# Sreyan88/audio-ssl

Measured on AMD Instinct MI355X. Metric: upstream clips/sec (1s@16kHz, 64-mel), higher is better.
Workload: dtype bf16; 1 GPU; delores-m upstream step (log-mel + 2 views + q/k conv encoders + MoCo + 3 Barlow heads + bwd + SGD), 1 s @ 16 kHz, 64 mel, batch 512/GPU, queue 65536; global_batch=512, parallelism=dp1

## Files before the change

### audio-ssl_amd/csrc/augment.hip

```cpp
#include "common.h"

namespace {

constexpr float F32_EPS = 1.1920928955078125e-07f;
constexpr float F32_MAX = 3.4028234663852886e+38f;

__global__ __launch_bounds__(256) void clip_moments_kernel(const float* __restrict__ x, double* __restrict__ mom, int n) {
    __shared__ double sh[16];
    const float* p = x + (long)blockIdx.x * n;
    double s = 0.0, q = 0.0;
    for (int i = threadIdx.x; i < n; i += 256) { const double v = p[i]; s += v; q += v * v; }
    s = block_sum(s, sh);
    q = block_sum(q, sh);
    if (threadIdx.x == 0) { mom[2 * blockIdx.x] = s; mom[2 * blockIdx.x + 1] = q; }
}

__device__ __forceinline__ float chain64(float v, float x_mine, double r_mine, float& keep) {
    const int rlo = __double2loint(r_mine), rhi = __double2hiint(r_mine);
#pragma unroll
    for (int c = 0; c < 64; ++c) {
        const float x = __int_as_float(__builtin_amdgcn_readlane(__float_as_int(x_mine), c));
        const double r = __hiloint2double(__builtin_amdgcn_readlane(rhi, c), __builtin_amdgcn_readlane(rlo, c));
        v = v + (float)((double)(x - v) * r);
        keep = ((int)(threadIdx.x & 63) == c) ? v : keep;
    }
    return v;
}

__global__ __launch_bounds__(128) void runnorm_scan_kernel(const double* __restrict__ mom, int B, int n_elem, long long* state_i,
                                                           float* state_f, float* __restrict__ mu_out, float* __restrict__ sd_out) {
    extern __shared__ __attribute__((aligned(16))) double sm[];
    double* rn = sm;
    float* m_s = reinterpret_cast<float*>(rn + B);
    float* mu_s = m_s + B;
    float* v_s = mu_s + B;
    float* s2_s = v_s + B;
    const long long n0 = state_i[0], max_update = state_i[1];
    const double inv = 1.0 / (double)n_elem;
    const int tid = threadIdx.x, wave = tid >> 6, lane = tid & 63;
    const bool big = n0 + B > (1 << 24);
    for (int c = tid; c < B; c += 128) {
        m_s[c] = (float)(mom[2 * c] * inv);
        const long long n = n0 + c;
        rn[c] = (n > 0 && n < max_update) ? (big ? (double)(float)n : 1.0 / (double)(float)n) : 0.0;
    }
    float mu = state_f[0], s2 = state_f[1];
    const bool first = n0 == 0 && max_update > 0;
    __syncthreads();
    const int nblk = (B + 63) / 64;
    for (int k = 0; k <= nblk; ++k) {
        if (wave == 0 && k < nblk) {
            const int c0 = 64 * k, c = c0 + lane;
            if (!big) {
                if (k == 0 && first) mu = m_s[0];
                float keep = 0.f;
                mu = chain64(mu, c < B ? m_s[c] : 0.f, c < B ? rn[c] : 0.0, keep);
                if (c < B) mu_s[c] = keep;
            } else if (lane == 0) {
                int i = c0;
                const int c1 = min(c0 + 64, B);
                if (i == 0 && first) { mu = m_s[0]; mu_s[0] = mu; i = 1; }
                for (; i < c1; ++i) { if (rn[i] != 0.0) mu = mu + (m_s[i] - mu) / (float)rn[i]; mu_s[i] = mu; }
            }
        }
        if (wave == 1 && k >= 1) {
            const int c0 = 64 * (k - 1), c1 = min(c0 + 64, B), c = c0 + lane;
            float v = 0.f;
            if (c < c1) {
                const double ex = mom[2 * c] * inv, ex2 = mom[2 * c + 1] * inv, mud = (double)mu_s[c];
                v = (float)(ex2 - 2.0 * mud * ex + mud * mud);
            }
            if (!big) {
                if (k == 1 && first) s2 = __int_as_float(__builtin_amdgcn_readlane(__float_as_int(v), 0));
                float keep = 0.f;
                s2 = chain64(s2, v, c < c1 ? rn[c] : 0.0, keep);
                if (c < c1) s2_s[c] = keep;
            } else {
                if (c < c1) v_s[c] = v;
                __threadfence_block();
                if (lane == 0) {
                    int i = c0;
                    if (i == 0 && first) { s2 = v_s[0]; s2_s[0] = s2; i = 1; }
                    for (; i < c1; ++i) { if (rn[i] != 0.0) s2 = s2 + (v_s[i] - s2) / (float)rn[i]; s2_s[i] = s2; }
                }
            }
        }
        __syncthreads();
    }
    for (int c = tid; c < B; c += 128) {
        mu_out[c] = mu_s[c];
        sd_out[c] = fminf(fmaxf(sqrtf(s2_s[c]), F32_EPS), F32_MAX);
    }
    if (tid == 0) {
        long long upd = max_update - n0;
        upd = upd < 0 ? 0 : (upd > B ? B : upd);
        state_i[0] = n0 + upd;
        state_f[0] = mu_s[B - 1];
        state_f[1] = s2_s[B - 1];
    }
}

__global__ __launch_bounds__(256) void aug_normalize_kernel(const float* __restrict__ x, const float* __restrict__ mu,
                                                            const float* __restrict__ sd, float* __restrict__ bank,
                                                            long slot0, int R, int n) {
    const int c = blockIdx.y;
    const float m = mu[c], s = sd[c];
    const float* src = x + (long)c * n;
    float* dst = bank + ((slot0 + c) % R) * (long)n;
    for (int i = blockIdx.x * 256 + threadIdx.x; i < n; i += gridDim.x * 256) dst[i] = (src[i] - m) / s;
}

__device__ __forceinline__ void cubic_coeffs(float t, float* c) {
    const float A = -0.75f;
    float x = t + 1.f;
    c[0] = ((A * x - 5.f * A) * x + 8.f * A) * x - 4.f * A;
    x = t;
    c[1] = ((A + 2.f) * x - (A + 3.f)) * x * x + 1.f;
    x = 1.f - t;
    c[2] = ((A + 2.f) * x - (A + 3.f)) * x * x + 1.f;
    x = x + 1.f;
    c[3] = ((A * x - 5.f * A) * x + 8.f * A) * x - 4.f * A;
}

struct ViewArgs {
    const float* bank; const int* ip; const float* fp; float* out1; float* out2;
    int F, T, canvas_h, canvas_w, y0, x0, log_mix;
};

__global__ __launch_bounds__(256) void aug_views_kernel(ViewArgs a) {
    extern __shared__ __attribute__((aligned(16))) float mixed[];
    const int c = blockIdx.x, view = blockIdx.y;
    const int* ip = a.ip + (c * 2 + view) * 8;
    const float* fp = a.fp + (c * 2 + view) * 2;
    const int n = a.F * a.T;
    const float* xs = a.bank + (long)ip[0] * n;
    const int partner = ip[1];
    if (partner >= 0) {
        const float* zs = a.bank + (long)partner * n;
        const float cs = fp[0], cp = fp[1];
        if (a.log_mix) {
            for (int i = threadIdx.x; i < n; i += 256) mixed[i] = logf(cs * expf(xs[i]) + cp * expf(zs[i]) + F32_EPS);
        } else {
            for (int i = threadIdx.x; i < n; i += 256) mixed[i] = cp * zs[i] + cs * xs[i];
        }
    } else {
        for (int i = threadIdx.x; i < n; i += 256) mixed[i] = xs[i];
    }
    __syncthreads();
    float* out = (view == 0 ? a.out1 : a.out2) + (long)c * n;
    if (!ip[6]) {
        for (int i = threadIdx.x; i < n; i += 256) out[i] = mixed[i];
        return;
    }
    const int ci = ip[2], cj = ip[3], h = ip[4], w = ip[5];
    const float sy = a.F > 1 ? (float)(h - 1) / (float)(a.F - 1) : 0.f;
    const float sx = a.T > 1 ? (float)(w - 1) / (float)(a.T - 1) : 0.f;
    for (int idx = threadIdx.x; idx < n; idx += 256) {
        const int oy = idx / a.T, ox = idx - oy * a.T;
        const float ry = sy * (float)oy, rx = sx * (float)ox;
        const float fy = floorf(ry), fx = floorf(rx);
        float wy[4], wx[4];
        cubic_coeffs(fminf(fmaxf(ry - fy, 0.f), 1.f), wy);
        cubic_coeffs(fminf(fmaxf(rx - fx, 0.f), 1.f), wx);
        const int iy = (int)fy, ix = (int)fx;
        int xi[4];
#pragma unroll
        for (int q = 0; q < 4; ++q) xi[q] = cj + min(max(ix - 1 + q, 0), w - 1) - a.x0;
        float acc = 0.f;
#pragma unroll
        for (int p = 0; p < 4; ++p) {
            const int yy = ci + min(max(iy - 1 + p, 0), h - 1) - a.y0;
            const bool rowin = yy >= 0 && yy < a.F;
            float row = 0.f;
#pragma unroll
            for (int q = 0; q < 4; ++q) {
                const bool in = rowin && xi[q] >= 0 && xi[q] < a.T;
                const float s = in ? mixed[yy * a.T + xi[q]] : 0.f;
                row = row + s * wx[q];
            }
            acc = acc + row * wy[p];
        }
        out[idx] = acc;
    }
}

__global__ __launch_bounds__(256) void mask_fill_kernel(float* __restrict__ x, const int* __restrict__ tab, int max_masks,
                                                        int F, int T, int zero_fill) {
    __shared__ double sh[16];
    float* p = x + (long)blockIdx.x * F * T;
    const int n = F * T;
    for (int k = 0; k < max_masks; ++k) {
        const int* e = tab + ((long)blockIdx.x * max_masks + k) * 4;
        const int axis = e[0], st = e[1], en = e[2];
        if (axis < 0) break;
        float fill = 0.f;
        if (!zero_fill) {
            double s = 0.0;
            for (int i = threadIdx.x; i < n; i += 256) s += (double)p[i];
            s = block_sum(s, sh);
            fill = (float)(s / (double)n);
        }
        __syncthreads();
        if (en > st) {
            if (axis == 1) {
                const int cnt = (en - st) * T;
                for (int i = threadIdx.x; i < cnt; i += 256) p[st * T + i] = fill;
            } else {
                const int wdt = en - st, cnt = wdt * F;
                for (int i = threadIdx.x; i < cnt; i += 256) { const int f = i / wdt, t = st + i - f * wdt; p[f * T + t] = fill; }
            }
        }
        __syncthreads();
    }
}

__global__ __launch_bounds__(256) void kmix_cluster_kernel(const float* __restrict__ views, const float* __restrict__ cent, int F, int T,
                                                           int K, int* __restrict__ cluster) {
    __shared__ float m[128];
    __shared__ float best_d[256];
    __shared__ int best_i[256];
    const float* x = views + (long)blockIdx.x * F * T;
    for (int f = threadIdx.x >> 2; f < F; f += 64) {
        float s = 0.f;
        for (int t = threadIdx.x & 3; t < T; t += 4) s += x[f * T + t];
        s += __shfl_xor(s, 1, 64);
        s += __shfl_xor(s, 2, 64);
        if ((threadIdx.x & 3) == 0) m[f] = s / (float)T;
    }
    __syncthreads();
    float bd = 3.0e38f;
    int bi = 0x7fffffff;
    for (int c = threadIdx.x; c < K; c += 256) {
        float d = 0.f;
        for (int f = 0; f < F; ++f) { const float e = m[f] - cent[c * F + f]; d += e * e; }
        if (d < bd) { bd = d; bi = c; }
    }
    best_d[threadIdx.x] = bd; best_i[threadIdx.x] = bi;
    __syncthreads();
    for (int o = 128; o > 0; o >>= 1) {
        if (threadIdx.x < o) {
            const float d2 = best_d[threadIdx.x + o];
            const int i2 = best_i[threadIdx.x + o];
            if (d2 < best_d[threadIdx.x] || (d2 == best_d[threadIdx.x] && i2 < best_i[threadIdx.x])) { best_d[threadIdx.x] = d2; best_i[threadIdx.x] = i2; }
        }
        __syncthreads();
    }
    if (threadIdx.x == 0) cluster[blockIdx.x] = best_i[0];
}

__global__ __launch_bounds__(256) void kmix_apply_kernel(const float* __restrict__ views, const float* __restrict__ ring,
                                                         const int* __restrict__ slot, const float* __restrict__ coef, int n,
                                                         int log_mix, float* __restrict__ out) {
    const int v = blockIdx.y;
    const int z = slot[v];
    const float cs = coef[2 * v], cp = coef[2 * v + 1];
    const float* x = views + (long)v * n;
    const float* zs = ring + (long)(z < 0 ? 0 : z) * n;
    float* o = out + (long)v * n;
    for (int i = blockIdx.x * 256 + threadIdx.x; i < n; i += gridDim.x * 256) {
        const float xv = x[i];
        if (z < 0) o[i] = xv;
        else o[i] = log_mix ? logf(cs * expf(xv) + cp * expf(zs[i]) + F32_EPS) : cp * zs[i] + cs * xv;
    }
}

}

extern "C" int audiossl_clip_moments(const float* x, double* mom, int B, int n, void* stream) {
    ASSL_REQUIRE(x && mom && B > 0 && n > 0);
    hipLaunchKernelGGL(clip_moments_kernel, dim3(B), dim3(256), 0, static_cast<hipStream_t>(stream), x, mom, n);
    ASSL_LAUNCH_CHECK();
}

extern "C" int audiossl_runnorm_scan(const double* mom, int B, int n_elem, long long* state_i, float* state_f,
                                     float* mu_out, float* sd_out, void* stream) {
    ASSL_REQUIRE(mom && state_i && state_f && mu_out && sd_out && B > 0 && B <= 3840 && n_elem > 0);
    const size_t dyn = (size_t)B * (sizeof(double) + 4 * sizeof(float));
    static bool attr_set = false;
    if (!attr_set) {
        if (hipFuncSetAttribute(reinterpret_cast<const void*>(runnorm_scan_kernel), hipFuncAttributeMaxDynamicSharedMemorySize,
                                96 * 1024) != hipSuccess) return ASSL_ELAUNCH;
        attr_set = true;
    }
    hipLaunchKernelGGL(runnorm_scan_kernel, dim3(1), dim3(128), dyn, static_cast<hipStream_t>(stream), mom, B, n_elem,
                       state_i, state_f, mu_out, sd_out);
    ASSL_LAUNCH_CHECK();
}

extern "C" int audiossl_aug_normalize(const float* x, const float* mu, const float* sd, float* bank, long slot0,
                                      int R, int B, int n, void* stream) {
    ASSL_REQUIRE(x && mu && sd && bank && R > 0 && B > 0 && B <= R && n > 0 && slot0 >= 0);
    hipLaunchKernelGGL(aug_normalize_kernel, dim3(ceil_div(n, 1024), B), dim3(256), 0, static_cast<hipStream_t>(stream),
                       x, mu, sd, bank, slot0, R, n);
    ASSL_LAUNCH_CHECK();
}

extern "C" int audiossl_aug_views(const float* bank, int R, const int* ip, const float* fp, float* out1, float* out2,
                                  int B, int F, int T, int canvas_h, int canvas_w, int log_mix, void* stream) {
    ASSL_REQUIRE(bank && ip && fp && out1 && out2 && B > 0 && F > 0 && T > 0 && R > 0);
    ASSL_REQUIRE(canvas_h >= F && canvas_w >= T && (size_t)F * T * 4 <= 60 * 1024);
    ViewArgs a{bank, ip, fp, out1, out2, F, T, canvas_h, canvas_w, (canvas_h - F) / 2, (canvas_w - T) / 2, log_mix};
    hipLaunchKernelGGL(aug_views_kernel, dim3(B, 2), dim3(256), (size_t)F * T * 4, static_cast<hipStream_t>(stream), a);
    ASSL_LAUNCH_CHECK();
}

extern "C" int audiossl_mask_fill(float* x, const int* tab, int n_img, int max_masks, int F, int T, int zero_fill,
                                  void* stream) {
    ASSL_REQUIRE(x && tab && n_img > 0 && max_masks > 0 && F > 0 && T > 0);
    hipLaunchKernelGGL(mask_fill_kernel, dim3(n_img), dim3(256), 0, static_cast<hipStream_t>(stream), x, tab, max_masks,
                       F, T, zero_fill);
    ASSL_LAUNCH_CHECK();
}

extern "C" int audiossl_kmix_cluster(const float* views, const float* centroids, int n_views, int F, int T, int K, int* cluster,
                                     void* stream) {
    ASSL_REQUIRE(views && centroids && cluster && n_views > 0 && F > 0 && F <= 128 && T > 0 && K > 0);
    hipLaunchKernelGGL(kmix_cluster_kernel, dim3(n_views), dim3(256), 0, static_cast<hipStream_t>(stream), views, centroids, F, T, K,
                       cluster);
    ASSL_LAUNCH_CHECK();
}

extern "C" int audiossl_kmix_apply(const float* views, const float* ring, const int* slot, const float* coef, int n_views, int n,
                                   int log_mix, float* out, void* stream) {
    ASSL_REQUIRE(views && ring && slot && coef && out && n_views > 0 && n > 0);
    hipLaunchKernelGGL(kmix_apply_kernel, dim3(ceil_div(n, 1024), n_views), dim3(256), 0, static_cast<hipStream_t>(stream), views,
                       ring, slot, coef, n, log_mix, out);
    ASSL_LAUNCH_CHECK();
}
```

### audio-ssl_amd/src/augmentations/augmentations.py

```python
import os
import random

import numpy as np
import torch
from torch import nn

from src import _native as N

__all__ = ["AugmentationModule", "RunningNorm", "MixupBYOLA", "RandomResizeCrop", "SpecAugment", "log_mixup_exp",
           "PrecomputedNorm", "NormalizeBatch"]

_F32 = np.float32


def log_mixup_exp(xa, xb, alpha):
    x = alpha * xa.exp() + (1.0 - alpha) * xb.exp()
    return torch.log(x + torch.finfo(x.dtype).eps)


class RunningNorm(nn.Module):

    def __init__(self, epoch_samples, max_update_epochs=10, axis=(1, 2)):
        super().__init__()
        self.max_update = int(epoch_samples * max_update_epochs)
        self.axis = list(axis)
        self.state_i = None
        self.state_f = None

    def device_state(self, device):
        if self.state_i is None:
            self.state_i = torch.tensor([0, self.max_update], dtype=torch.int64, device=device)
            self.state_f = torch.zeros(2, dtype=torch.float32, device=device)
        return self.state_i, self.state_f

    def __len__(self):
        return 0 if self.state_i is None else int(self.state_i[0])

    @property
    def mean(self):
        return None if self.state_f is None else self.state_f[0]

    @property
    def std(self):
        if self.state_f is None:
            return None
        return torch.clamp(torch.sqrt(self.state_f[1]), torch.finfo().eps, torch.finfo().max)

    def __repr__(self):
        return self.__class__.__name__ + f"(max_update={self.max_update},axis={self.axis})"


class MixupBYOLA(nn.Module):
    def __init__(self, ratio=0.4, n_memory=2048, log_mixup_exp=True):
        super().__init__()
        self.ratio, self.n, self.log_mixup_exp = ratio, n_memory, log_mixup_exp

    def __repr__(self):
        return self.__class__.__name__ + f"(ratio={self.ratio},n={self.n},log_mixup_exp={self.log_mixup_exp})"


class RandomResizeCrop(nn.Module):
    def __init__(self, virtual_crop_scale=(1.0, 1.5), freq_scale=(0.6, 1.5), time_scale=(0.6, 1.5)):
        super().__init__()
        assert time_scale[1] >= 1.0 and freq_scale[1] >= 1.0
        self.virtual_crop_scale, self.freq_scale, self.time_scale = virtual_crop_scale, freq_scale, time_scale
        self.interpolation = "bicubic"

    @staticmethod
    def get_params(virtual_crop_size, in_size, time_scale, freq_scale):
        canvas_h, canvas_w = virtual_crop_size
        src_h, src_w = in_size
        h = int(np.clip(int(np.random.uniform(*freq_scale) * src_h), 1, canvas_h))
        w = int(np.clip(int(np.random.uniform(*time_scale) * src_w), 1, canvas_w))
        i = random.randint(0, canvas_h - h) if canvas_h > h else 0
        j = random.randint(0, canvas_w - w) if canvas_w > w else 0
        return i, j, h, w

    def __repr__(self):
        s = self.__class__.__name__ + f"(virtual_crop_size={self.virtual_crop_scale}"
        s += ", time_scale={0}".format(tuple(round(v, 4) for v in self.time_scale))
        return s + ", freq_scale={0})".format(tuple(round(v, 4) for v in self.freq_scale))


class Kmix(nn.Module):

    def __init__(self, ratio=0.4, n_memory=2048, log_mixup_exp=True, top_k=None, centroid_path=None, centroids=None):
        super().__init__()
        self.ratio, self.n, self.log_mixup_exp, self.top_k = ratio, n_memory, log_mixup_exp, top_k
        c = centroids if centroids is not None else torch.load(centroid_path, map_location="cpu", weights_only=True)
        self.centroids = torch.as_tensor(c, dtype=torch.float32).cpu()
        cn = self.centroids / self.centroids.norm(dim=-1, keepdim=True)
        self.far_order = torch.topk(torch.cdist(cn, cn, p=2), k=len(cn), dim=1).indices.numpy()
        self._cn = cn.contiguous()
        self.bank_ids = []
        self.entries = 0
        self.ring = self.R = None
        self.last_choice = None
        self.draws = []

    def __repr__(self):
        return self.__class__.__name__ + f"(ratio={self.ratio},n={self.n},log_mixup_exp={self.log_mixup_exp})"

    def _ensure(self, n_new, numel, dev):
        need = self.n + max(n_new, 2)
        if self.ring is None or self.ring.device != dev or self.ring.shape[1] != numel or need > self.R:
            old, old_R = self.ring, self.R
            self.R = max(need, self.R or 0)
            self.ring = torch.zeros(self.R, numel, dtype=torch.float32, device=dev)
            if old is not None and old.shape[1] == numel:
                for g in range(max(0, self.entries - len(self.bank_ids)), self.entries):
                    self.ring[g % self.R].copy_(old[g % old_R])
            self._cn_dev = self._cn.to(dev)

    def _select(self, cx):
        nb = len(self.bank_ids)
        if nb >= 128:
            if nb < self.top_k:
                raise TypeError("list indices must be integers or slices, not NoneType")
            ids = np.asarray(self.bank_ids)
            for cid in self.far_order[cx]:
                l = np.nonzero(ids == cid)[0]
                if len(l):
                    break
            l = l[:128]
            k = int(np.random.randint(len(l)))
            self.draws.append((len(l), k))
            return int(l[k])
        k = int(np.random.randint(nb))
        self.draws.append((nb, k))
        return k

    def _plan_call(self, cx, slot_out, coef_out, i):
        alpha = self.ratio * np.random.random()
        nb = len(self.bank_ids)
        if nb:
            j = self._select(cx)
            slot_out[i] = (self.entries - nb + j) % self.R
            a1 = 1.0 - alpha
            coef_out[i] = (_F32(a1), _F32(1.0 - a1))
            self.last_choice = j
        else:
            slot_out[i] = -1
            self.last_choice = None
        self.bank_ids.append(int(cx))
        if len(self.bank_ids) > self.n:
            self.bank_ids.pop(0)
        self.entries += 1

    @torch.no_grad()
    def mix_batch(self, views):
        if not views.is_cuda:
            raise RuntimeError("Kmix runs on the GPU only (no CPU fallback)")
        views = views.contiguous().float()
        n, F, T = views.shape
        dev = views.device
        self._ensure(n, F * T, dev)
        ids_d = torch.empty(n, dtype=torch.int32, device=dev)
        N.call("kmix_cluster", views, self._cn_dev, n, F, T, self._cn.shape[0], ids_d)
        g0 = self.entries
        flat = views.view(n, F * T)
        first = g0 % self.R
        k = min(n, self.R - first)
        self.ring[first:first + k].copy_(flat[:k])
        if k < n:
            self.ring[:n - k].copy_(flat[k:])
        ids = ids_d.cpu().numpy()
        slot = np.full(n, -1, np.int32)
        coef = np.zeros((n, 2), _F32)
        for i in range(n):
            self._plan_call(ids[i], slot, coef, i)
        out = torch.empty_like(views)
        N.call("kmix_apply", views, self.ring, torch.from_numpy(slot).to(dev), torch.from_numpy(coef).to(dev), n, F * T,
               int(bool(self.log_mixup_exp)), out)
        return out

    def forward(self, x):
        src = x.device
        out = self.mix_batch((x if x.is_cuda else x.cuda()).reshape(1, x.shape[-2], x.shape[-1]))
        return out if src.type == "cuda" else out.to(src)


class SpecAugment(nn.Module):

    def __init__(self, F=30, T=40, num_freq_masks=2, num_time_masks=2, replace_with_zero=False):
        super().__init__()
        self.F, self.T, self.nf, self.nt, self.zero = F, T, num_freq_masks, num_time_masks, replace_with_zero

    def plan(self, n_mel, n_time):
        out = []
        for axis, width, size, count in ((1, self.F, n_mel, self.nf), (0, self.T, n_time, self.nt)):
            for _ in range(count):
                f = random.randrange(0, width)
                f0 = random.randrange(0, size - f)
                if f == 0:
                    break
                end = random.randrange(f0, f0 + f)
                out.append((axis, f0, end))
        return out

    @property
    def max_masks(self):
        return self.nf + self.nt


class PrecomputedNorm(nn.Module):
    def __init__(self, stats, axis=(1, 2)):
        super().__init__()
        self.axis = list(axis)
        self.mean, self.std = stats

    def forward(self, X):
        return (X - self.mean) / self.std


class NormalizeBatch(nn.Module):
    def __init__(self, axis=(0, 2, 3)):
        super().__init__()
        self.axis = list(axis)

    def forward(self, X):
        m = X.mean(dim=self.axis, keepdims=True)
        s = torch.clamp(X.std(dim=self.axis, keepdims=True), torch.finfo().eps, torch.finfo().max)
        return (X - m) / s


class AugmentationModule:

    def __init__(self, config, len_of_files, max_batch=1024):
        aug = config["pretrain"]["augmentations"]
        self.mix = self.rrc = self.spec = None
        if "MixupBYOLA" in aug:
            self.mix = MixupBYOLA(ratio=aug["MixupBYOLA"]["ratio"], log_mixup_exp=aug["MixupBYOLA"]["log_mixup_exp"])
        if "RandomResizeCrop" in aug:
            r = aug["RandomResizeCrop"]
            self.rrc = RandomResizeCrop(virtual_crop_scale=r["virtual_crop_scale"], freq_scale=r["freq_crop_scale"],
                                        time_scale=r["time_crop_scale"])
        if "SpecAugment" in aug:
            self.spec = SpecAugment(**aug["SpecAugment"])
        self.kmix = None
        if "Kmix" in aug:
            k = aug["Kmix"]
            self.kmix = Kmix(ratio=k["ratio"], log_mixup_exp=k["log_mixup_exp"], top_k=k["top_k"], centroid_path=k.get("centroid_path"),
                             centroids=k.get("centroids"))
        if "PatchDrop" in aug:
            raise NotImplementedError("PatchDrop is not part of the HIP two-view path (SURVEY 2.4); drop the key")
        self.train_transform = nn.Sequential(*[m for m in (self.mix, self.rrc, self.kmix, self.spec) if m is not None])
        self.pre_norm = None
        if config["pretrain"]["normalization"] == "mean_var":
            self.pre_norm = RunningNorm(epoch_samples=2 * len_of_files)
        self.n_memory = self.mix.n if self.mix is not None else 0
        self.max_batch = max_batch
        self.n_entries = 0
        self.clips_seen = 0
        self.bank = None
        self.R = 0
        self.last_plan = None

    def plan(self, B, F, T, lens=None, unit=0):
        import ctypes
        ip = np.zeros((B, 2, 8), np.int32)
        fp = np.zeros((B, 2, 2), _F32)
        K = self.spec.max_masks if self.spec is not None else 1
        mk = np.full((B, 2, K, 4), -1, np.int32)
        ch = cw = 0
        if self.rrc is not None:
            ch, cw = int(F * self.rrc.virtual_crop_scale[0]), int(T * self.rrc.virtual_crop_scale[1])
        lens_a = None if lens is None else np.ascontiguousarray(lens, dtype=np.int32)
        starts = np.zeros(B, np.int32)
        st = np.random.get_state()
        np_key = np.ascontiguousarray(st[1], dtype=np.uint32)
        np_pos = ctypes.c_int(int(st[2]))
        ps = random.getstate()
        py_key = np.array(ps[1][:624], dtype=np.uint32)
        py_pos = ctypes.c_int(int(ps[1][624]))
        ne = ctypes.c_longlong(self.n_entries)
        fs = self.rrc.freq_scale if self.rrc is not None else (1.0, 1.0)
        ts = self.rrc.time_scale if self.rrc is not None else (1.0, 1.0)
        sp = self.spec
        N.call_host("aug_plan_host", np_key.ctypes.data, ctypes.addressof(np_pos), py_key.ctypes.data,
                    ctypes.addressof(py_pos), B, F, T, self.clips_seen, ctypes.addressof(ne), self.R, self.n_memory,
                    int(self.mix is not None), float(self.mix.ratio) if self.mix is not None else 0.0,
                    int(self.rrc is not None), float(fs[0]), float(fs[1]), float(ts[0]), float(ts[1]), ch, cw,
                    int(sp is not None), sp.F if sp else 1, sp.T if sp else 1, sp.nf if sp else 0, sp.nt if sp else 0,
                    lens_a.ctypes.data if lens_a is not None else None, int(unit), starts.ctypes.data, ip.ctypes.data,
                    fp.ctypes.data, mk.ctypes.data)
        self.last_starts = starts if lens_a is not None else None
        np.random.set_state((st[0], np_key, np_pos.value, st[3], st[4]))
        random.setstate((ps[0], tuple(int(v) for v in py_key) + (py_pos.value,), ps[2]))
        self.n_entries = ne.value
        self.clips_seen += B
        masks = []
        if sp is not None:
            for b in range(B):
                for v in range(2):
                    masks.append([tuple(int(x) for x in m[:3]) for m in mk[b, v] if m[0] >= 0])
        return ip, fp, (ch, cw), masks

    def plan_py(self, B, F, T, lens=None, unit=0):
        starts = np.zeros(B, np.int32)
        ip = np.zeros((B, 2, 8), np.int32)
        fp = np.zeros((B, 2, 2), _F32)
        masks = []
        ch = cw = 0
        if self.rrc is not None:
            ch, cw = int(F * self.rrc.virtual_crop_scale[0]), int(T * self.rrc.virtual_crop_scale[1])
        for b in range(B):
            c = self.clips_seen + b
            if lens is not None:
                over = int(lens[b]) - unit
                starts[b] = random.randint(0, over) if over > 0 else 0
            for v in range(2):
                e = ip[b, v]
                e[0] = c % self.R
                e[1] = -1
                if self.mix is not None:
                    alpha = self.mix.ratio * np.random.random()
                    n_bank = min(self.n_entries, self.n_memory)
                    if n_bank > 0:
                        k = np.random.randint(n_bank)
                        g = self.n_entries - n_bank + k
                        e[1] = (g // 2) % self.R
                        a1 = 1.0 - alpha
                        fp[b, v, 0] = _F32(a1)
                        fp[b, v, 1] = _F32(1.0 - a1)
                    self.n_entries += 1
                if self.rrc is not None:
                    i, j, h, w = RandomResizeCrop.get_params((ch, cw), (F, T), self.rrc.time_scale, self.rrc.freq_scale)
                    e[2:7] = (i, j, h, w, 1)
                if self.spec is not None:
                    masks.append(self.spec.plan(F, T))
        self.clips_seen += B
        self.last_starts = starts if lens is not None else None
        return ip, fp, (ch, cw), masks

    def _ensure_ring(self, B, n=None, device=None):
        need = 1025 + max(B, self.max_batch)
        if self.R == 0:
            self.R = need
        elif need > self.R:
            if self.bank is not None:
                old, old_R = self.bank, self.R
                self.bank = torch.zeros(need, old.shape[1], dtype=torch.float32, device=old.device)
                for c in range(max(0, self.clips_seen - 1025), self.clips_seen):
                    self.bank[c % need].copy_(old[c % old_R])
            self.R = need
        self.max_batch = max(self.max_batch, B)
        if self.bank is None and n is not None:
            self.bank = torch.zeros(self.R, n, dtype=torch.float32, device=device)

    def _upload(self, key, arr, dev, depth=int(os.environ.get("AUDIOSSL_UPLOAD_DEPTH", "2"))):
        ring = self.__dict__.setdefault("_staging", {}).setdefault((key, arr.shape, arr.dtype.str), {"i": 0, "slots": []})
        if len(ring["slots"]) < depth:
            ring["slots"].append([torch.from_numpy(np.empty_like(arr)).pin_memory(), None])
        slot = ring["slots"][ring["i"] % len(ring["slots"])]
        ring["i"] += 1
        if slot[1] is not None:
            slot[1].synchronize()
        slot[0].numpy()[...] = arr
        out = slot[0].to(dev, non_blocking=True)
        slot[1] = torch.cuda.Event()
        slot[1].record()
        return out

    def _ensure_bank(self, B, n, device):
        self._ensure_ring(B, n, device)

    @torch.no_grad()
    def augment_batch(self, lms, plan=None):
        if lms.dim() == 4:
            lms = lms[:, 0]
        lms = lms.contiguous().float()
        if not lms.is_cuda:
            raise RuntimeError("AugmentationModule runs on the GPU only (no CPU fallback)")
        B, F, T = lms.shape
        n = F * T
        dev = lms.device
        self._ensure_bank(B, n, dev)
        mu = torch.zeros(B, dtype=torch.float32, device=dev)
        sd = torch.ones(B, dtype=torch.float32, device=dev)
        if self.pre_norm is not None:
            mom = torch.empty(B, 2, dtype=torch.float64, device=dev)
            si, sf = self.pre_norm.device_state(dev)
            N.call("clip_moments", lms, mom, B, n)
            N.call("runnorm_scan", mom, B, n, si, sf, mu, sd)
        if plan is None:
            slot0 = self.clips_seen % self.R
            plan = self.plan(B, F, T)
        else:
            slot0 = int(plan[0][0, 0, 0])
        N.call("aug_normalize", lms, mu, sd, self.bank, slot0, self.R, B, n)
        ip, fp, (ch, cw), masks = plan
        self.last_plan = (ip, fp, masks)
        ip_d = self._upload("ip", ip, dev)
        fp_d = self._upload("fp", fp, dev)
        v1 = torch.empty(B, 1, F, T, dtype=torch.float32, device=dev)
        v2 = torch.empty(B, 1, F, T, dtype=torch.float32, device=dev)
        log_mix = 1 if (self.mix is None or self.mix.log_mixup_exp) else 0
        N.call("aug_views", self.bank, self.R, ip_d, fp_d, v1, v2, B, F, T, max(ch, F), max(cw, T), log_mix)
        if self.kmix is not None:
            both = torch.stack([v1[:, 0], v2[:, 0]], dim=1).reshape(2 * B, F, T)
            mixed = self.kmix.mix_batch(both).view(B, 2, F, T)
            v1, v2 = mixed[:, 0:1].contiguous(), mixed[:, 1:2].contiguous()
        if self.spec is not None:
            K = self.spec.max_masks
            tab = np.full((B, 2, K, 4), -1, np.int32)
            for idx, ms in enumerate(masks):
                for k, (axis, st, en) in enumerate(ms):
                    tab[idx // 2, idx % 2, k] = (axis, st, en, 0)
            for v, view in enumerate((v1, v2)):
                t = self._upload(f"mask{v}", np.ascontiguousarray(tab[:, v]), dev)
                N.call("mask_fill", view, t, B, K, F, T, int(self.spec.zero))
        return v1, v2

    def __call__(self, x):
        src = x.device
        v1, v2 = self.augment_batch(x.cuda() if not x.is_cuda else x)
        v1, v2 = v1[0], v2[0]
        return (v1, v2) if src.type == "cuda" else (v1.to(src), v2.to(src))
```

### include/audiossl_hip.h

```cpp
#ifndef AUDIOSSL_HIP_H
#define AUDIOSSL_HIP_H

#include <stdint.h>

#ifdef __cplusplus
extern "C" {
#endif

#define AUDIOSSL_OK 0
#define AUDIOSSL_EINVAL (-1)
#define AUDIOSSL_ELAUNCH (-2)
#define AUDIOSSL_EALIGN (-3)

int audiossl_logmel_fwd(const float* wave, float* out, int B, int L, int T, int n_fft, int hop, int n_mels, int taps,
                        const float* win, const float* tw, const float* melw, const int* mel_start, float eps_pow,
                        float eps_log, int apply_log, void* stream);

int audiossl_fbank_fwd(const float* wave, const int* lens, const int* partner, const float* lam, float* clip_mean,
                       const int* bands, const int* bands_host, float* out, int B, int Lmax, int win_len, int shift, int n_fft, int n_mels,
                       int taps, int T_target, const float* win, const float* tw, const float* melw, const int* mel_start,
                       float preemph, float eps_log, float mean, float std, int skip_norm, int time_major, void* stream);

int audiossl_clip_moments(const float* x, double* mom, int B, int n, void* stream);
int audiossl_runnorm_scan(const double* mom, int B, int n_elem, long long* state_i, float* state_f, float* mu_out,
                          float* sd_out, void* stream);
int audiossl_aug_normalize(const float* x, const float* mu, const float* sd, float* bank, long slot0, int R, int B, int n,
                           void* stream);
int audiossl_aug_views(const float* bank, int R, const int* ip, const float* fp, float* out1, float* out2, int B, int F,
                       int T, int canvas_h, int canvas_w, int log_mix, void* stream);
int audiossl_aug_plan_host(uint32_t* np_key, int* np_pos, uint32_t* py_key, int* py_pos, int B, int F, int T,
                           long long clips_seen, long long* n_entries, int R, int n_memory, int use_mix, double ratio,
                           int use_rrc, double fs_lo, double fs_hi, double ts_lo, double ts_hi, int canvas_h,
                           int canvas_w, int use_spec, int spec_F, int spec_T, int spec_nf, int spec_nt, const int* lens,
                           int unit, int* starts, int* ip, float* fp, int* masks);

int audiossl_resample_sinc(const float* x, float* y, int clips, int n_orig, int n_out, const int* n, const int* off_l,
                           const int* off_r, const double* eta_l, const double* eta_r, const double* win, const double* delta,
                           int nwin, int index_step, void* stream);

int audiossl_pcm_window(const void* pcm, long pcm_bytes, const long long* tab, const long long* tab_host, float* out, int B,
                        int unit, int align, void* stream);

int audiossl_kmix_cluster(const float* views, const float* centroids, int n_views, int F, int T, int K, int* cluster,
                          void* stream);
int audiossl_kmix_apply(const float* views, const float* ring, const int* slot, const float* coef, int n_views, int n,
                        int log_mix, float* out, void* stream);
int audiossl_mask_fill(float* x, const int* tab, int n_img, int max_masks, int F, int T, int zero_fill, void* stream);

int audiossl_conv1_stats(const float* img, int N, int F, int T, const float* w, const float* bias, const float* gamma,
                         const float* beta, float* running_mean, float* running_var, float momentum, float eps,
                         double* mom, float* scale, float* shift, float* save_mean, float* save_rstd, void* stream);
#define AUDIOSSL_CONV1_XL_PARTS 4
int audiossl_conv1_fwd(int dtype, const float* img, int N, int F, int T, const float* w, const float* bias,
                       const float* scale, const float* shift, void* out, float* xl, void* stream);
#define AUDIOSSL_CONV1_MOM_SLOT (17 * 54)
int audiossl_conv1_moments_pair(const float* img_a, const float* img_b, int N, int F, int T, double* mom, void* stream);
int audiossl_conv1_fwd_train(const float* img, int N, int F, int T, double* mom, double count, const float* w, const float* bias,
                             const float* gamma, const float* beta, float* running_mean, float* running_var, float momentum,
                             float eps, float* scale, float* shift, float* save_mean, float* save_rstd, void* out, float* xl,
                             void* stream);
int audiossl_conv1_bwd(int dtype, int conv_dtype, const float* img, int N, int F, int T, const float* w, const float* bias,
                       const float* gamma, const float* scale, const float* shift, const float* mean, const float* rstd,
                       const double* mom, const void* dP, const void* dxl, float* acc, float* dW, float* dbias,
                       float* dgamma, float* dbeta, void* stream);

int audiossl_colstats(int dtype, const void* x, int groups, long M, int C, long ld, int want_sq, double* sum,
                      double* sumsq, void* stream);
int audiossl_bn_finalize(const double* sum, const double* sumsq, int groups, double count, int C, const float* gamma,
                         const float* beta, float* running_mean, float* running_var, float momentum, float eps,
                         float* scale, float* shift, float* save_mean, float* save_rstd, void* stream);
int audiossl_bn_relu_pool_fwd(int dtype, int ydtype, const void* Y, const float* scale, const float* shift, void* P, int N,
                              int Ti, int Fi, void* stream);
int audiossl_bn_relu_pool_train_fwd(int dtype, int ydtype, const void* Y, const double* sum, const double* sumsq, int stat_replicas,
                                    double count, const float* gamma, const float* beta, float* running_mean, float* running_var,
                                    float momentum, float eps, void* P, float* scale, float* shift, float* save_mean, float* save_rstd,
                                    int N, int Ti, int Fi, void* stream);
int audiossl_bn_relu_pooled_fwd(int dtype, const void* Praw, const float* scale, const float* shift, void* P, int N, int To, int Fo,
                                void* stream);
int audiossl_bn_relu_pooled_train_fwd(int dtype, const void* Praw, const double* sum, const double* sumsq, int stat_replicas,
                                      double count, const float* gamma, const float* beta, float* running_mean, float* running_var,
                                      float momentum, float eps, void* P, float* scale, float* shift, float* save_mean,
                                      float* save_rstd, int N, int To, int Fo, void* stream);
int audiossl_tmean_fwd(int dtype, int out_f32, const void* P, void* xl, int N, int To, int Fo, void* stream);
int audiossl_tmean3_fwd(int dtype, int out_f32, const void* P1, void* x1, const float* x1_parts, int To1, int Fo1, const void* P2,
                        void* x2, int To2, int Fo2, const void* P3, void* x3, int To3, int Fo3, int N, void* stream);
int audiossl_bn_relu_pool_bwd(int dtype, int ydtype, int gdtype, const void* Y, const void* dP, const void* dxl, const float* scale,
                              const float* shift, const float* mean, const float* rstd, float* stat, void* dY,
                              float* dgamma, float* dbeta, int N, int Ti, int Fi, void* stream);
int audiossl_bn_relu_pool_bwd_p(int dtype, int ydtype, int gdtype, const void* Y, const void* P, const void* dP, const void* dxl,
                                const float* scale, const float* shift, const float* mean, const float* rstd, float* stat, void* dY,
                                float* dgamma, float* dbeta, int N, int Ti, int Fi, void* stream);
int audiossl_conv1_moments(const float* img, int N, int F, int T, double* mom, void* stream);
int audiossl_conv1_finalize(double* mom_totals, const float* w, const float* bias, const float* gamma, const float* beta,
                            float* running_mean, float* running_var, float momentum, float eps, double count, float* scale,
                            float* shift, float* save_mean, float* save_rstd, void* stream);
int audiossl_conv1_bwd_sums(int dtype, int conv_dtype, const float* img, int N, int F, int T, const float* w, const float* bias,
                            const float* gamma, const float* scale, const float* shift, const float* mean, const float* rstd,
                            const double* mom, const void* dP, const void* dxl, float* acc, float* lstat, void* stream);
int audiossl_conv1_bwd_finalize(const float* acc, const double* mom, const float* w, const float* bias, const float* gamma,
                                const float* mean, const float* rstd, double count_global, const float* gstat, float* dW,
                                float* dbias, float* dgamma, float* dbeta, void* stream);
int audiossl_bn_relu_pool_bwd_stats(int dtype, int ydtype, int gdtype, const void* Y, const void* dP, const void* dxl,
                                    const float* scale, const float* shift, const float* mean, const float* rstd, float* stat,
                                    int N, int Ti, int Fi, void* stream);
int audiossl_bn_relu_pool_bwd_apply(int dtype, int ydtype, int gdtype, const void* Y, const void* dP, const void* dxl,
                                    const float* scale, const float* shift, const float* mean, const float* rstd, float* stat,
                                    const float* gstat, double count_global, void* dY, float* dgamma, float* dbeta, int N, int Ti,
                                    int Fi, void* stream);
int audiossl_colbn_bwd_stats(int dtype, int adtype, int gdtype, const void* a, const void* dh, const float* scale,
                             const float* shift, const float* mean, const float* rstd, int relu, int groups, long M, int C,
                             double* tmp, void* stream);
int audiossl_colbn_bwd_apply(int dtype, int adtype, int gdtype, const void* a, const void* dh, const float* scale,
                             const float* shift, const float* mean, const float* rstd, int relu, int groups, long M, int C,
                             const double* sums, double count, void* da, void* stream);
int audiossl_im2col3x3(int dtype, const void* X, void* col, int N, int Ti, int Fi, void* stream);
int audiossl_pack_conv_w(int dtype, const float* W, void* Wf, void* Wd, void* stream);
int audiossl_pack_conv_w2(int dtype, const float* Wa, void* Wfa, void* Wda, const float* Wb, void* Wfb, void* Wdb, void* stream);
int audiossl_unpack_conv_dw(const float* dWp, float* dW, void* stream);

int audiossl_conv3x3_fwd(const void* X, const void* W, const float* bias, void* Y, int out_f32, double* sum,
                         double* sumsq, int stat_replicas, int N, int Ti, int Fi, void* stream);
int audiossl_conv3x3_pool_fwd(const void* X, const void* W, const float* bias, const float* gamma, void* Y, void* Praw, double* sum,
                              double* sumsq, int stat_replicas, int N, int Ti, int Fi, void* stream);
int audiossl_conv3x3_wgrad(const void* dY, const void* X, float* dWp, float* workspace, long workspace_floats, int N, int Ti,
                           int Fi, void* stream);

int audiossl_gemm(int dtype, int trans_a, int trans_b, int M, int N, int K, float alpha, const void* A, long lda,
                  const void* B, long ldb, void* C, long ldc, const float* bias, int relu, const uint8_t* keep, long ldk,
                  float keep_scale, const void* gate, long ldg, int out_f32, int atomic, int ksplit, const float* resid,
                  long ldr, void* stream);

int audiossl_gemm_dropout(int trans_a, int trans_b, int M, int N, int K, float alpha, const void* A, long lda, const void* B,
                          long ldb, void* C, long ldc, const float* bias, int relu, unsigned long long seed, float p,
                          const long long* counter, float keep_scale, void* stream);

int audiossl_gemm_multi(int count, int trans_a, int trans_b, int M, const int* N, const int* K, float alpha,
                        const void* const* A, const long* lda, const void* const* B, const long* ldb, void* const* C,
                        const long* ldc, int out_f32, int atomic, int ksplit, void* stream);
int audiossl_gemm_multi_sgd(int count, int trans_a, int trans_b, int M, const int* Nv, const int* K, float alpha,
                            const void* const* A, const long* lda, const void* const* B, const long* ldb, float* const* P,
                            float* const* Mom, void* const* Shadow, const long* ldp, float lr, float momentum, float weight_decay,
                            float grad_scale, const float* grad_scale_dev, void* stream);
int audiossl_gemm_multi_barlow(int count, int D, const int* K, float alpha, const void* const* A, const long* lda,
                               const void* const* B, const long* ldb, void* const* dc, const float* coef, const float* dscale,
                               float* const* loss_rep, void* stream);

int audiossl_maxmean_fwd(int dtype, int out_f32, const void* H, void* y, uint8_t* arg, int N, int Tt, int D, void* stream);
int audiossl_maxmean_bwd(int dtype, int gdtype, const void* dy, const uint8_t* arg, const void* H, void* dA, int N, int Tt,
                         int D, void* stream);

int audiossl_colbn_fwd(int dtype, int adtype, const void* a, const float* scale, const float* shift, int relu, void* h,
                       int groups, long M, int C, void* stream);
int audiossl_colbn_train_fwd(int dtype, int adtype, const void* a, const float* gamma, const float* beta,
                             float* running_mean, float* running_var, float momentum, float eps, int relu, int groups,
                             long M, int C, void* h, float* scale, float* shift, float* save_mean, float* save_rstd,
                             void* stream);
int audiossl_colbn_bwd(int dtype, int adtype, int gdtype, const void* a, const void* dh, const float* scale, const float* shift, const float* mean,
                       const float* rstd, int relu, int groups, long M, int C, double* tmp, void* da, float* dgamma,
                       float* dbeta, void* stream);
int audiossl_colbn_train_fwd_multi(int count, int adtype, const void* const* a, const float* const* gamma,
                                   const float* const* beta, float* const* running_mean, float* const* running_var,
                                   float momentum, float eps, int relu, int groups, long M, int C, void* const* h,
                                   float* const* stats, void* stream);
int audiossl_colbn_bwd_multi(int count, int adtype, int gdtype, const void* const* a, const void* const* dh,
                             const float* const* stats, int relu, int groups, long M, int C, void* const* da,
                             float* const* dgamma, float* const* dbeta, void* stream);
int audiossl_barlow_loss_multi(int count, const float* const* c, int D, const float* coef, const float* dscale,
                               void* const* dc, float* const* loss_out, void* stream);
int audiossl_add_d2f(const double* src, float* dst, int n, void* stream);
int audiossl_barlow_loss(int dtype, const float* c, int D, float coef, float dscale, void* dc, float* loss_out,
                         void* stream);

int audiossl_l2norm_fwd(int dtype, const float* q, int B, int D, void* qn, float* qn32, float* inv_norm, void* stream);
int audiossl_moco_prep(int dtype, const float* q, const float* k, int B, int D, float scale, void* qn, float* qn32, float* qinv,
                       void* kn, float* kn32, float* kinv, float* lpos, void* stream);
int audiossl_rowdot(const float* a, const float* b, int B, int D, float scale, float* out, void* stream);
int audiossl_moco_ce_fwd(const float* lpos, const float* lneg, int B, int K, float* lse, float* loss_out, void* stream);
int audiossl_moco_ce_bwd(int dtype, const float* lpos, const float* lneg, const float* lse, int B, int K, float gscale,
                         void* P, float* dlpos, void* stream);
int audiossl_moco_logits(int mode, const void* qn, const void* queue, int B, int K, int dim, float inv_t, float* part,
                         const float* lse, float gscale, void* P, void* stream);
int audiossl_moco_lse_merge(const float* lpos, const float* part, int B, int nslot, float gscale, float* lse,
                            float* loss_out, float* dlpos, void* stream);
int audiossl_l2norm_bwd(int dtype, const float* dqn, const float* dlpos, const float* kn32, const float* qn32,
                        const float* inv_norm, int B, int D, void* dq, void* stream);
int audiossl_enqueue(int dtype, const float* keys, int B, int D, int K, int ptr, long long* ptr_dev, float* queue, void* shadow,
                     void* stream);
int audiossl_ema_update(float* pk, const float* pq, long n, float m, void* shadow, void* stream);

int audiossl_set_prezeroed(int on);
int audiossl_last_kernel(char* name, int capacity);

int audiossl_sgd_momentum(float* p, float* g, float* buf, long n, float lr, float momentum, float weight_decay,
                          int first, float grad_scale, const float* grad_scale_dev, void* shadow_bf16, int zero_grad,
                          void* stream);
int audiossl_sgd_momentum_segments(float* p, float* g, float* buf, const long* segs, int nseg, long max_n, float lr, float momentum,
                                   float weight_decay, int first, float grad_scale, const float* grad_scale_dev, void* shadow_bf16,
                                   int zero_grad, void* stream);
int audiossl_zero_segments(float* g, const long* segs, int nseg, long max_n, void* stream);
int audiossl_cast(int dtype, const float* src, void* dst, long n, void* stream);
int audiossl_cast_back(int dtype, const void* src, float* dst, long n, void* stream);
int audiossl_dropout_mask(uint8_t* keep, long n, unsigned long long seed, float p, const long long* counter, void* stream);
int audiossl_relu_bwd(int dtype, const void* g, const void* h, void* out, long n, void* stream);
int audiossl_bn_eval_affine(const float* gamma, const float* beta, const float* running_mean, const float* running_var,
                            float eps, int C, float* scale, float* shift, void* stream);
int audiossl_axpy(float* y, const float* x, float a, long n, void* stream);
int audiossl_split_bf16(const float* x, void* hi, void* lo, long n, void* stream);
int audiossl_center_cast(const float* y, void* yc, float* cmean, int groups, long M, int C, void* stream);
int audiossl_shift_running_mean(const void* W, const float* cmean, float* running_mean, int D, int K, int groups,
                                float momentum, void* stream);
int audiossl_center_cast_multi(int count, const float* const* y, void* const* yc, float* const* cmean, const int* C, int groups,
                               long M, void* stream);
int audiossl_shift_running_mean_multi(int count, const void* const* W, const float* const* cmean, float* const* running_mean,
                                      int D, const int* K, int groups, float momentum, void* stream);

int audiossl_ntxent_fwd(const float* sim, int N, int B, float* lse, float* loss_out, void* stream);
int audiossl_ntxent_bwd(int dtype, const float* sim, const float* lse, int N, int B, float gscale, void* dsim, void* stream);

int audiossl_row_argmax(const float* dot, long N, int K, long long* assign, void* stream);
int audiossl_kmeans_accumulate(const float* x, const long long* assign, long N, int K, int D, float* sums, int* counts,
                               void* stream);
int audiossl_kmeans_update(const float* sums, const int* counts, int K, int D, float* centroids, void* stream);
int audiossl_kmeans_update_mean(const float* sums, const int* counts, int K, int D, float* centroids, void* stream);
int audiossl_row_sqnorm(const float* x, int rows, int D, float scale, float* out, void* stream);
int audiossl_ce_rows(int dtype, const float* logits, const long long* target, int B, int K, int ignore_index, int* cnt,
                     float* loss_out, void* dlogits, void* stream);

int audiossl_unfused_loss(int gdtype, const float* z1, const float* z2, const float* z3, const float* t,
                          const long long* label, int B, int C, long ld, float alpha, float beta, float gamma,
                          float* loss4, void* dz1, void* dz2, void* dz3, void* dt, void* stream);

int audiossl_knn_workspace(int Nq, long Nb, int k, long* bytes);
int audiossl_knn_topk(const void* q, const void* bank, int Nq, long Nb, int D, int k, float* top_sim, int* top_idx,
                      void* workspace, long workspace_bytes, void* stream);
int audiossl_knn_vote(const float* top_sim, const int* top_idx, const long long* bank_label, int Nq, int k, long Nb,
                      float inv_t, long long* pred, float* conf, void* stream);

int audiossl_cka_workspace(int n, int p, int q, long* bytes);
int audiossl_cka_center(const float* x, int n, int p, float* out, void* stream);
int audiossl_cka_sigma2(const float* x, int n, int p, double* sigma2, long long* count, void* workspace,
                        long workspace_bytes, void* stream);
int audiossl_cka_hsic(const float* x, const float* y, int n, int p, int q, int kernel, double sigma,
                      const double* sigma2_x, const double* sigma2_y, double* out, double* rowsum_k,
                      double* rowsum_l, void* workspace, long workspace_bytes, void* stream);

int audiossl_knn_graph_workspace(int n, int k, long* bytes);
int audiossl_knn_graph_l2(const float* x, int n, int d, int k, int* idx, float* d2, void* workspace, long workspace_bytes,
                          void* stream);
int audiossl_pic_workspace(int n, int k, long* bytes);
int audiossl_pic_build(const int* idx, const float* d2, int n, int k, double sigma, int* rowptr, int* col, double* w, int* nnz,
                       void* workspace, long workspace_bytes, void* stream);
int audiossl_pic_power(const int* rowptr, const int* col, const double* w, int n, long cap, double alpha, int iters, double* v,
                       void* workspace, long workspace_bytes, void* stream);
int audiossl_pic_assign(const int* rowptr, const int* col, const double* w, const double* v, int n, long cap, int* label,
                        int* count, void* workspace, long workspace_bytes, void* stream);

int audiossl_bce_rows(int dtype, const float* logits, const float* targets, long N, int C, float* loss_out, void* dlogits,
                      void* stream);
int audiossl_tagging_workspace(long N, int C, long* bytes);
int audiossl_tagging_stats(const float* scores, const unsigned char* targets, long N, int C, int* npos, long long* auc_num2,
                           double* ap, double* auc, void* workspace, long workspace_bytes, void* stream);

int audiossl_softmax_rows_fwd(const float* x, float* y, int M, int C, void* stream);
int audiossl_softmax_rows_bwd(const float* y, const float* gy, float* gx, int M, int C, void* stream);

int audiossl_attn_fwd(const void* qkv, void* out, float* lse, int B, int S, int H, float scale, void* stream);
int audiossl_attn_bwd(const void* qkv, const void* out, const void* dout, const float* lse, void* dqkv, int B, int S, int H,
                      float scale, void* stream);
int audiossl_layernorm_fwd(const float* x, const float* gamma, const float* beta, void* y, float* y32, float* mean, float* rstd,
                           int M, int C, float eps, void* stream);
int audiossl_layernorm_bwd(const float* dy, const float* x, const float* mean, const float* rstd, const float* gamma,
                           float* dres, float* dgamma, float* dbeta, int M, int C, void* stream);
int audiossl_gelu_fwd(const void* a, void* h, long n, void* stream);
int audiossl_gelu_bwd(const void* a, const void* dh, void* da, long n, void* stream);
int audiossl_patch_unfold(const float* x, void* out, int B, int F, int T, int fstride, int tstride, void* stream);
int audiossl_tile_rows(const float* src, float* out, long rows, int period, int group, float scale, int C, void* stream);
int audiossl_adamw(float* p, const float* g, float* m, float* v, long n, float lr, float beta1, float beta2, float eps,
                   float weight_decay, float grad_scale, const long long* step, void* stream);

int audiossl_mvit_pool_fwd(const void* qkv, int ldq, int col0, const float* w, const float* gamma, const float* beta, float* out,
                           float* z, float* mean, float* rstd, int B, int heads, int d, int H, int W, int Ho, int Wo, int sh, int sw,
                           float eps, void* stream);
int audiossl_mvit_pool_bwd(const void* qkv, int ldq, int col0, const float* w, const float* gamma, const float* dout, const float* z,
                           const float* mean, const float* rstd, float* dz, float* dw, float* dgamma, float* dbeta, void* dqkv, int B,
                           int heads, int d, int H, int W, int Ho, int Wo, int sh, int sw, void* stream);
int audiossl_mvit_attn_fwd(const float* q, const float* k, const float* v, const float* rh, const float* rw, const int* ih,
                           const int* iw, void* out, float* lse, int B, int heads, int d, int qh, int qw, int kh, int kw, int nrh,
                           int nrw, int residual, float scale, void* stream);
int audiossl_mvit_attn_bwd(const float* q, const float* k, const float* v, const float* rh, const float* rw, const int* ih,
                           const int* iw, const void* dout, const float* lse, float* dq, float* dk, float* dv, float* drh, float* drw,
                           int B, int heads, int d, int qh, int qw, int kh, int kw, int nrh, int nrw, int residual, float scale,
                           void* stream);
int audiossl_tokpool_max_fwd(const float* x, float* y, void* arg, int B, int H, int W, int C, int kh, int kw, int sh, int sw,
                             void* stream);
int audiossl_tokpool_max_bwd(const float* dy, const void* arg, float* dx, int B, int H, int W, int C, int kh, int kw, int sh, int sw,
                             void* stream);

int audiossl_lars_step(float* p, const float* g, float* mu, const void* seg, int n_seg, const float* lr, float weight_decay,
                       float momentum, float eta, float grad_scale, double* norms, void* stream);
int audiossl_larc_step(float* p, const float* g, float* mu, const void* seg, int n_seg, float lr, float weight_decay,
                       float momentum, float trust_coefficient, float eps, int clip, float grad_scale, double* norms,
                       void* stream);

#ifdef __cplusplus
}
#endif
#endif
```

Measured before the change: 273,100 clips/s.

## Restrict augmentation mixing to crop rectangle and precompute bicubic tap tables

The views kernel now mixes only the source pixels that the random-resize crop actually reads, writing them into a padded LDS image with a zero guard row and column. It also precomputes per-row and per-column bicubic weights and byte offsets once per block, so the inner loop drops the clamping and bounds checks. When no crop is applied, the mix is written straight to the output, skipping the LDS round trip and the resample. The old kernel stays available through an environment variable and a separate entry point, and the Python side skips allocating unused mu/sd zero and one tensors. Explicit fma ordering is used to try to keep results bitwise compatible with the old kernel.

```diff
diff --git a/audio-ssl_amd/csrc/augment.hip b/audio-ssl_amd/csrc/augment.hip
--- a/audio-ssl_amd/csrc/augment.hip
+++ b/audio-ssl_amd/csrc/augment.hip
@@ -127,7 +127,7 @@
     int F, T, canvas_h, canvas_w, y0, x0, log_mix;
 };
 
-__global__ __launch_bounds__(256) void aug_views_kernel(ViewArgs a) {
+__global__ __launch_bounds__(256) void aug_views_v1_kernel(ViewArgs a) {
     extern __shared__ __attribute__((aligned(16))) float mixed[];
     const int c = blockIdx.x, view = blockIdx.y;
     const int* ip = a.ip + (c * 2 + view) * 8;
@@ -184,6 +184,152 @@
     }
 }
 
+struct AugRect { int r0, r1, c0, c1; };
+
+__host__ __device__ inline AugRect aug_views_rect(int F, int T, int y0, int x0, int ci, int cj, int h, int w) {
+    AugRect r;
+    if (F == 1 && h > 3) h = 3;
+    if (T == 1 && w > 3) w = 3;
+    r.r0 = ci - y0 > 0 ? ci - y0 : 0;
+    r.r1 = ci + h - y0 < F ? ci + h - y0 : F;
+    r.c0 = cj - x0 > 0 ? cj - x0 : 0;
+    r.c1 = cj + w - x0 < T ? cj + w - x0 : T;
+    if (r.r1 <= r.r0 || r.c1 <= r.c0) r.r0 = r.r1 = r.c0 = r.c1 = 0;
+    return r;
+}
+
+__device__ __forceinline__ bool v1_mix_in_remainder(int i, int n) { return i + 256 >= n && ((i >> 8) & 1) == 0; }
+
+template <int MODE>
+__device__ __forceinline__ float mix_v1(float x, float z, float cs, float cp, bool remainder) {
+#pragma clang fp contract(off)
+    if (MODE == 2) {
+        const float ex = expf(x), t = cp * expf(z);
+        const float s = remainder ? cs * ex + t : __fmaf_rn(cs, ex, t);
+        return logf(s + F32_EPS);
+    }
+    if (MODE == 1) {
+        const float t = cs * x;
+        return remainder ? cp * z + t : __fmaf_rn(cp, z, t);
+    }
+    return x;
+}
+
+template <int MODE>
+__device__ __forceinline__ void mix_rect(const float* __restrict__ xs, const float* __restrict__ zs, float cs, float cp,
+                                         const AugRect rc, int T, int n, float* dst, int ld) {
+    const int rw = rc.c1 - rc.c0, cnt = (rc.r1 - rc.r0) * rw;
+    if (cnt <= 0) return;
+    const int dq = 256 / rw, dr = 256 - dq * rw;
+    const int r = (int)threadIdx.x / rw;
+    int col = (int)threadIdx.x - r * rw;
+    int i = (rc.r0 + r) * T + rc.c0 + col, o = (rc.r0 + r) * ld + rc.c0 + col;
+#pragma unroll 4
+    for (int e = threadIdx.x; e < cnt; e += 256) {
+        dst[o] = mix_v1<MODE>(xs[i], MODE ? zs[i] : 0.f, cs, cp, v1_mix_in_remainder(i, n));
+        col += dr; i += dq * T + dr; o += dq * ld + dr;
+        if (col >= rw) { col -= rw; i += T - rw; o += ld - rw; }
+    }
+}
+
+__device__ __forceinline__ void mix_rect_mode(int mode, const float* __restrict__ xs, const float* __restrict__ zs, float cs,
+                                              float cp, const AugRect rc, int T, int n, float* dst, int ld) {
+    if (mode == 2) mix_rect<2>(xs, zs, cs, cp, rc, T, n, dst, ld);
+    else if (mode == 1) mix_rect<1>(xs, zs, cs, cp, rc, T, n, dst, ld);
+    else mix_rect<0>(xs, zs, cs, cp, rc, T, n, dst, ld);
+}
+
+__device__ __forceinline__ void cubic_coeffs_v1(float t, float* c) {
+#pragma clang fp contract(off)
+    const float A = -0.75f;
+    float x = t + 1.f;
+    c[0] = __fmaf_rn(__fmaf_rn(__fmaf_rn(A, x, -(5.f * A)), x, 8.f * A), x, -(4.f * A));
+    x = t;
+    c[1] = __fmaf_rn(__fmaf_rn(A + 2.f, x, -(A + 3.f)) * x, x, 1.f);
+    x = 1.f - t;
+    c[2] = __fmaf_rn(__fmaf_rn(A + 2.f, x, -(A + 3.f)) * x, x, 1.f);
+    x = x + 1.f;
+    c[3] = __fmaf_rn(__fmaf_rn(__fmaf_rn(A, x, -(5.f * A)), x, 8.f * A), x, -(4.f * A));
+}
+
+__device__ __forceinline__ void tap_entry(int o, int size, int c0, int len, int org, int lim, int stride, int guard,
+                                          float4* w_out, int4* off_out) {
+#pragma clang fp contract(off)
+    const float sc = size > 1 ? (float)(len - 1) / (float)(size - 1) : 0.f;
+    const float r = sc * (float)o;
+    const float f = floorf(r);
+    float w[4];
+    cubic_coeffs_v1(fminf(fmaxf(r - f, 0.f), 1.f), w);
+    const int i0 = (int)f;
+    int off[4];
+#pragma unroll
+    for (int k = 0; k < 4; ++k) {
+        const int v = c0 + min(max(i0 - 1 + k, 0), len - 1) - org;
+        off[k] = (v >= 0 && v < lim) ? v * stride : guard;
+    }
+    *w_out = make_float4(w[0], w[1], w[2], w[3]);
+    *off_out = make_int4(off[0], off[1], off[2], off[3]);
+}
+
+__device__ __forceinline__ float lds_at(const float* img, int byte_off) {
+    return *reinterpret_cast<const float*>(reinterpret_cast<const char*>(img) + byte_off);
+}
+
+__device__ __forceinline__ float tap_row(const float* img, int ry, const float4 wx, const int4 cx) {
+#pragma clang fp contract(off)
+    float row = __fmaf_rn(lds_at(img, ry + cx.x), wx.x, 0.f);
+    row = __fmaf_rn(lds_at(img, ry + cx.y), wx.y, row);
+    row = __fmaf_rn(lds_at(img, ry + cx.z), wx.z, row);
+    return __fmaf_rn(lds_at(img, ry + cx.w), wx.w, row);
+}
+
+__device__ __forceinline__ float tap_sum(const float* img, const float4 wy, const int4 ry, const float4 wx, const int4 cx) {
+#pragma clang fp contract(off)
+    float acc = __fmaf_rn(tap_row(img, ry.x, wx, cx), wy.x, 0.f);
+    acc = __fmaf_rn(tap_row(img, ry.y, wx, cx), wy.y, acc);
+    acc = __fmaf_rn(tap_row(img, ry.z, wx, cx), wy.z, acc);
+    return __fmaf_rn(tap_row(img, ry.w, wx, cx), wy.w, acc);
+}
+
+__global__ __launch_bounds__(256) void aug_views_kernel(ViewArgs a) {
+    extern __shared__ __attribute__((aligned(16))) float img[];
+    const int c = blockIdx.x, view = blockIdx.y;
+    const int* ip = a.ip + (c * 2 + view) * 8;
+    const float* fp = a.fp + (c * 2 + view) * 2;
+    const int F = a.F, T = a.T, n = F * T, tid = threadIdx.x;
+    const float* xs = a.bank + (long)ip[0] * n;
+    const int partner = ip[1];
+    const float* zs = a.bank + (long)(partner >= 0 ? partner : 0) * n;
+    const float cs = fp[0], cp = fp[1];
+    float* out = (view == 0 ? a.out1 : a.out2) + (long)c * n;
+    const int mode = partner < 0 ? 0 : (a.log_mix ? 2 : 1);
+    if (!ip[6]) {
+        mix_rect_mode(mode, xs, zs, cs, cp, AugRect{0, F, 0, T}, T, n, out, T);
+        return;
+    }
+    const int ci = ip[2], cj = ip[3], h = ip[4], w = ip[5];
+    const int S = T + 1;
+    mix_rect_mode(mode, xs, zs, cs, cp, aug_views_rect(F, T, a.y0, a.x0, ci, cj, h, w), T, n, img, S);
+    const int guard_row = F * S;
+    float4* roww = reinterpret_cast<float4*>(img + (((F + 1) * S + 3) & ~3));
+    int4* rowo = reinterpret_cast<int4*>(roww + F);
+    float4* colw = reinterpret_cast<float4*>(rowo + F);
+    int4* colo = reinterpret_cast<int4*>(colw + T);
+    for (int k = tid; k < F + S; k += 256) img[k < F ? k * S + T : guard_row + k - F] = 0.f;
+    for (int k = tid; k < F + T; k += 256) {
+        if (k < F) tap_entry(k, F, ci, h, a.y0, F, S * 4, guard_row * 4, roww + k, rowo + k);
+        else tap_entry(k - F, T, cj, w, a.x0, T, 4, T * 4, colw + k - F, colo + k - F);
+    }
+    __syncthreads();
+    const int dq = 256 / T, dr = 256 - dq * T;
+    int oy = tid / T, ox = tid - oy * T;
+    for (int idx = tid; idx < n; idx += 256) {
+        out[idx] = tap_sum(img, roww[oy], rowo[oy], colw[ox], colo[ox]);
+        oy += dq; ox += dr;
+        if (ox >= T) { ox -= T; ++oy; }
+    }
+}
+
 __global__ __launch_bounds__(256) void mask_fill_kernel(float* __restrict__ x, const int* __restrict__ tab, int max_masks,
                                                         int F, int T, int zero_fill) {
     __shared__ double sh[16];
@@ -295,13 +441,42 @@
     ASSL_LAUNCH_CHECK();
 }
 
-extern "C" int audiossl_aug_views(const float* bank, int R, const int* ip, const float* fp, float* out1, float* out2,
-                                  int B, int F, int T, int canvas_h, int canvas_w, int log_mix, void* stream) {
+namespace {
+
+int launch_aug_views(bool v1, const float* bank, int R, const int* ip, const float* fp, float* out1, float* out2, int B, int F,
+                     int T, int canvas_h, int canvas_w, int log_mix, void* stream) {
     ASSL_REQUIRE(bank && ip && fp && out1 && out2 && B > 0 && F > 0 && T > 0 && R > 0);
     ASSL_REQUIRE(canvas_h >= F && canvas_w >= T && (size_t)F * T * 4 <= 60 * 1024);
     ViewArgs a{bank, ip, fp, out1, out2, F, T, canvas_h, canvas_w, (canvas_h - F) / 2, (canvas_w - T) / 2, log_mix};
-    hipLaunchKernelGGL(aug_views_kernel, dim3(B, 2), dim3(256), (size_t)F * T * 4, static_cast<hipStream_t>(stream), a);
-    ASSL_LAUNCH_CHECK();
+    const size_t lds = ((((size_t)(F + 1) * (T + 1) + 3) & ~(size_t)3) + (size_t)(F + T) * 8) * 4;
+    const hipStream_t st = static_cast<hipStream_t>(stream);
+    if (v1 || lds > 64 * 1024) hipLaunchKernelGGL(aug_views_v1_kernel, dim3(B, 2), dim3(256), (size_t)F * T * 4, st, a);
+    else hipLaunchKernelGGL(aug_views_kernel, dim3(B, 2), dim3(256), lds, st, a);
+    ASSL_LAUNCH_CHECK();
+}
+
+}
+
+extern "C" int audiossl_aug_views(const float* bank, int R, const int* ip, const float* fp, float* out1, float* out2,
+                                  int B, int F, int T, int canvas_h, int canvas_w, int log_mix, void* stream) {
+    static const int v1_only = getenv("AUDIOSSL_AUG_V1") ? atoi(getenv("AUDIOSSL_AUG_V1")) : 0;
+    return launch_aug_views(v1_only != 0, bank, R, ip, fp, out1, out2, B, F, T, canvas_h, canvas_w, log_mix, stream);
+}
+
+extern "C" int audiossl_aug_views_v1(const float* bank, int R, const int* ip, const float* fp, float* out1, float* out2,
+                                     int B, int F, int T, int canvas_h, int canvas_w, int log_mix, void* stream) {
+    return launch_aug_views(true, bank, R, ip, fp, out1, out2, B, F, T, canvas_h, canvas_w, log_mix, stream);
+}
+
+extern "C" int audiossl_aug_views_rect_host(const int* ip, int n_plans, int F, int T, int canvas_h, int canvas_w, int* rect) {
+    ASSL_REQUIRE(ip && rect && n_plans > 0 && F > 0 && T > 0 && canvas_h >= F && canvas_w >= T);
+    for (int k = 0; k < n_plans; ++k) {
+        const int* e = ip + (long)k * 8;
+        AugRect r{0, F, 0, T};
+        if (e[6]) r = aug_views_rect(F, T, (canvas_h - F) / 2, (canvas_w - T) / 2, e[2], e[3], e[4], e[5]);
+        rect[4 * k] = r.r0; rect[4 * k + 1] = r.r1; rect[4 * k + 2] = r.c0; rect[4 * k + 3] = r.c1;
+    }
+    return ASSL_OK;
 }
 
 extern "C" int audiossl_mask_fill(float* x, const int* tab, int n_img, int max_masks, int F, int T, int zero_fill,
diff --git a/audio-ssl_amd/src/augmentations/augmentations.py b/audio-ssl_amd/src/augmentations/augmentations.py
--- a/audio-ssl_amd/src/augmentations/augmentations.py
+++ b/audio-ssl_amd/src/augmentations/augmentations.py
@@ -376,13 +376,16 @@
         n = F * T
         dev = lms.device
         self._ensure_bank(B, n, dev)
-        mu = torch.zeros(B, dtype=torch.float32, device=dev)
-        sd = torch.ones(B, dtype=torch.float32, device=dev)
         if self.pre_norm is not None:
+            mu = torch.empty(B, dtype=torch.float32, device=dev)
+            sd = torch.empty(B, dtype=torch.float32, device=dev)
             mom = torch.empty(B, 2, dtype=torch.float64, device=dev)
             si, sf = self.pre_norm.device_state(dev)
             N.call("clip_moments", lms, mom, B, n)
             N.call("runnorm_scan", mom, B, n, si, sf, mu, sd)
+        else:
+            mu = torch.zeros(B, dtype=torch.float32, device=dev)
+            sd = torch.ones(B, dtype=torch.float32, device=dev)
         if plan is None:
             slot0 = self.clips_seen % self.R
             plan = self.plan(B, F, T)
diff --git a/include/audiossl_hip.h b/include/audiossl_hip.h
--- a/include/audiossl_hip.h
+++ b/include/audiossl_hip.h
@@ -28,6 +28,9 @@
                            void* stream);
 int audiossl_aug_views(const float* bank, int R, const int* ip, const float* fp, float* out1, float* out2, int B, int F,
                        int T, int canvas_h, int canvas_w, int log_mix, void* stream);
+int audiossl_aug_views_v1(const float* bank, int R, const int* ip, const float* fp, float* out1, float* out2, int B, int F,
+                          int T, int canvas_h, int canvas_w, int log_mix, void* stream);
+int audiossl_aug_views_rect_host(const int* ip, int n_plans, int F, int T, int canvas_h, int canvas_w, int* rect);
 int audiossl_aug_plan_host(uint32_t* np_key, int* np_pos, uint32_t* py_key, int* py_pos, int B, int F, int T,
                            long long clips_seen, long long* n_entries, int R, int n_memory, int use_mix, double ratio,
                            int use_rrc, double fs_lo, double fs_hi, double ts_lo, double ts_hi, int canvas_h,
```

After: 273,400 clips/s, median of 6. No clear change (+0.1%).
